# azuxmioy/Render-In-Between

Measured on AMD Instinct MI355X. Metric: rendered frames/sec at 512x512 (generator forward + blend, device-resident), higher is better.
Workload: dtype f32

## Files before the change

### render-in-between_amd/csrc/kernels.hip.h

```cpp
#pragma once
#include "igemm.hip.h"

namespace rib {

struct GemmDmaParams {
  const float* A; const float* B; float* C;
  int M, N, K, lda, ldc;
  size_t sA, sB, sC;
  int modB;
  int K2; unsigned long long kmask;
};

typedef uint32_t u32x4 __attribute__((ext_vector_type(4)));
__device__ __forceinline__ void split3_bf16(const float4 p, const float4 q, bf16x8& hi, bf16x8& mid, bf16x8& lo) {
  const float x[8] = {p.x, p.y, p.z, p.w, q.x, q.y, q.z, q.w};
  u32x4 h, m, l;
#pragma unroll
  for (int i = 0; i < 4; ++i) {
    const uint32_t u0 = __float_as_uint(x[2 * i]), u1 = __float_as_uint(x[2 * i + 1]);
    h[i] = __builtin_amdgcn_perm(u1, u0, 0x07060302u);
    const float r0 = x[2 * i] - __uint_as_float(u0 & 0xffff0000u), r1 = x[2 * i + 1] - __uint_as_float(u1 & 0xffff0000u);
    const uint32_t v0 = __float_as_uint(r0), v1 = __float_as_uint(r1);
    m[i] = __builtin_amdgcn_perm(v1, v0, 0x07060302u);
    const float s0 = r0 - __uint_as_float(v0 & 0xffff0000u), s1 = r1 - __uint_as_float(v1 & 0xffff0000u);
// ... 281 lines not shown
  const float* beta;
};

__device__ __forceinline__ void block_stats_64(const StatSrc& s, int n, int c0, int nch, double* red ,
                                               float* s_sc, float* s_sh) {
  const int j = threadIdx.x & 63, q = threadIdx.x >> 6;
  double a1 = 0.0, a2 = 0.0;
  if (j < nch) stats_from_partials(s.part + (size_t)n * s.tiles * 2 * s.Cs, s.tiles, s.Cs, c0 + j, q, 4, a1, a2);
  red[(q * 64 + j) * 2] = a1; red[(q * 64 + j) * 2 + 1] = a2;
  __syncthreads();
  if (q == 0 && j < nch) {
    double t1 = 0.0, t2 = 0.0;
#pragma unroll
    for (int k = 0; k < 4; ++k) { t1 += red[(k * 64 + j) * 2]; t2 += red[(k * 64 + j) * 2 + 1]; }
    float sc, sh;
    scale_shift_of(t1, t2, s.inv_count, s.gamma ? s.gamma[c0 + j] : 1.f, s.beta ? s.beta[c0 + j] : 0.f, sc, sh);
    s_sc[j] = sc; s_sh[j] = sh;
  }
  __syncthreads();
}

enum { WSRC_PLAIN = 0, WSRC_SPADE = 1, WSRC_JOIN = 2 };
struct WinoInParams {
  const float* x; int H, W, xC, Cin;
  const float* pro_scale; const float* pro_shift; int pro_ld, pro_lrelu;
  StatSrc st;
  float* v; int tilesY, tilesX;
  int nslices, ublocks;
  int x_ups; const float* slab; int slab_ld, col0; const float* sbias;
  const float* x2; const float* xres; float* o; const float* pro2_scale; const float* pro2_shift; StatSrc st2;
  int ldv;
  int nslices2, Cin2, xC2, x2_ups, lrelu2, pro2_ld;
  const float* slab2; int slab2_ld, col0_2; const float* sbias2;
};
__device__ __forceinline__ WinoInParams wino_second(const WinoInParams& p) {
  WinoInParams q = p;
  q.x = p.x2; q.xC = p.xC2; q.Cin = p.Cin2; q.x_ups = p.x2_ups; q.pro_lrelu = p.lrelu2;
  q.pro_scale = p.pro2_scale; q.pro_shift = p.pro2_shift; q.pro_ld = p.pro2_ld; q.st = p.st2;
  q.slab = p.slab2; q.slab_ld = p.slab2_ld; q.col0 = p.col0_2; q.sbias = p.sbias2;
  q.x2 = nullptr; q.v = p.v + p.Cin;
  return q;
}

__device__ __forceinline__ float spade_mod1(float x, float sc, float sh, float g, float bg, float b, float bb) {
  return fmaf(fmaf(x, sc, sh), 1.f + (g + bg), b + bb);
}

template <int MODE> struct WinoConsts { float4 sc, sh, bg, bb, sc2, sh2; bool aff; };
template <int MODE> struct WinoRaw { float4 a, b, c; };

template <int MODE>
__device__ __forceinline__ void wino_in_consts(const WinoInParams& p, int n, int slice, int c4, bool cok, double* red, float* s_sc,
                                               float* s_sh, WinoConsts<MODE>& k) {
  k.sc = make_float4(1.f, 1.f, 1.f, 1.f); k.sh = make_float4(0.f, 0.f, 0.f, 0.f);
  k.aff = false;
  const int l = (threadIdx.x & 15) * 4;
  if (p.st.part) {
    block_stats_64(p.st, n, slice * 64, min(64, p.Cin - slice * 64), red, s_sc, s_sh);
    k.sc = make_float4(s_sc[l], s_sc[l + 1], s_sc[l + 2], s_sc[l + 3]);
    k.sh = make_float4(s_sh[l], s_sh[l + 1], s_sh[l + 2], s_sh[l + 3]);
    k.aff = true;
  } else if (p.pro_scale && cok) {
    k.sc = *reinterpret_cast<const float4*>(p.pro_scale + (size_t)n * p.pro_ld + c4 * 4);
    k.sh = *reinterpret_cast<const float4*>(p.pro_shift + (size_t)n * p.pro_ld + c4 * 4);
    k.aff = true;
  }
// ... 128 lines not shown
  int nslices, ublocks;
};

__device__ __forceinline__ void wino_out_partials(double (*red)[256][4], const double s1[4], const double s2[4], double* stat_part,
                                                  int n, int ublocks, int ub, int slice, int CoutPad) {
#pragma unroll
  for (int e = 0; e < 4; ++e) { red[0][threadIdx.x][e] = s1[e]; red[1][threadIdx.x][e] = s2[e]; }
  __syncthreads();
  if (threadIdx.x < 64) {
    const int c = slice * 64 + threadIdx.x;
    if (c < CoutPad) {
      const int g = threadIdx.x >> 2, e = threadIdx.x & 3;
      double a1 = 0.0, a2 = 0.0;
#pragma unroll
      for (int s = 0; s < 16; ++s) { a1 += red[0][s * 16 + g][e]; a2 += red[1][s * 16 + g][e]; }
      double* dst = stat_part + (((size_t)n * ublocks + ub) * 2) * CoutPad;
      dst[c] = a1;
      dst[CoutPad + c] = a2;
    }
  }
}

__global__ __launch_bounds__(256) void k_wino_out(const WinoOutParams p) {
  __shared__ __attribute__((aligned(16))) double red[2][256][4];
  const int c4n = p.CoutPad / 4;
  const int slice = blockIdx.x % p.nslices, ub = blockIdx.x / p.nslices;
  const int c4 = slice * 16 + (threadIdx.x & 15);
  const int n = blockIdx.y;
  const int ntiles = p.tilesY * p.tilesX;
  double s1[4] = {0.0, 0.0, 0.0, 0.0}, s2[4] = {0.0, 0.0, 0.0, 0.0};
  if (c4 < c4n) {
    const float4 bv = *reinterpret_cast<const float4*>(p.bias + c4 * 4);
    const size_t plane = (size_t)ntiles * p.CoutPad;
    for (int u = ub * 16 + (threadIdx.x >> 4); u < ntiles * 2; u += p.ublocks * 16) {
      const int r = u & 1, tile = u >> 1;
      const float* mb = p.m + (size_t)n * 16 * plane + (size_t)tile * p.CoutPad + c4 * 4;
      float4 mm[3][4];
#pragma unroll
      for (int a = 0; a < 3; ++a)
#pragma unroll
        for (int q = 0; q < 4; ++q) mm[a][q] = *reinterpret_cast<const float4*>(mb + (size_t)((r + a) * 4 + q) * plane);
      const float sg = r ? -1.f : 1.f;
      float4 uu[4];
#pragma unroll
      for (int q = 0; q < 4; ++q)
        uu[q] = make_float4(mm[0][q].x + sg * (mm[1][q].x + mm[2][q].x), mm[0][q].y + sg * (mm[1][q].y + mm[2][q].y),
                            mm[0][q].z + sg * (mm[1][q].z + mm[2][q].z), mm[0][q].w + sg * (mm[1][q].w + mm[2][q].w));
      float4 yv[2];
      yv[0] = RIB_F4_ADD(RIB_F4_ADD(uu[0], uu[1]), uu[2]);
      yv[1] = RIB_F4_SUB(RIB_F4_SUB(uu[1], uu[2]), uu[3]);
      const int ty = tile / p.tilesX, tx = tile % p.tilesX;
      const int oy = 2 * ty + r;
      float rr[2][4];
#pragma unroll
      for (int q = 0; q < 2; ++q) {
        const int cy = min(oy, p.Hout - 1), cx = min(2 * tx + q, p.Wout - 1);
#pragma unroll
        for (int e = 0; e < 4; ++e)
          rr[q][e] = p.res ? p.res[(((size_t)n * p.Hout + cy) * p.Wout + cx) * p.resC + min(c4 * 4 + e, p.resC - 1)] : 0.f;
      }
#pragma unroll
      for (int q = 0; q < 2; ++q) {
        const int ox = 2 * tx + q;
        const bool inb = oy < p.Hout && ox < p.Wout;
        const float v4[4] = {yv[q].x + bv.x, yv[q].y + bv.y, yv[q].z + bv.z, yv[q].w + bv.w};
#pragma unroll
        for (int e = 0; e < 4; ++e) {
          float t = apply_act(v4[e] + rr[q][e], p.act);
          const bool ok = inb && c4 * 4 + e < p.Cout;
          if (ok) p.y[(((size_t)n * p.Hout + oy) * p.Wout + ox) * p.yC + p.yoff + c4 * 4 + e] = t;
          t = ok ? t : 0.f;
          s1[e] += (double)t; s2[e] += (double)t * (double)t;
        }
      }
    }
  }
  if (p.stat_part) wino_out_partials(red, s1, s2, p.stat_part, n, p.ublocks, ub, slice, p.CoutPad);
}

__device__ __constant__ float kWino4BT[6][6] = {
    {81.f / 64, 0.f, -45.f / 16, 0.f, 1.f, 0.f},        {0.f, -27.f / 16, -9.f / 4, 3.f / 4, 1.f, 0.f},
    {0.f, 27.f / 16, -9.f / 4, -3.f / 4, 1.f, 0.f},     {0.f, -27.f / 32, -9.f / 16, 3.f / 2, 1.f, 0.f},
    {0.f, 27.f / 32, -9.f / 16, -3.f / 2, 1.f, 0.f},    {0.f, 81.f / 64, 0.f, -45.f / 16, 0.f, 1.f}};
__device__ __constant__ float kWino4AT[4][6] = {
    {1.f, 1.f, 1.f, 1.f, 1.f, 0.f},                      {0.f, 3.f / 4, -3.f / 4, 3.f / 2, -3.f / 2, 0.f},
    {0.f, 9.f / 16, 9.f / 16, 9.f / 4, 9.f / 4, 0.f},    {0.f, 27.f / 64, -27.f / 64, 27.f / 8, -27.f / 8, 1.f}};

__device__ __forceinline__ float4 f4_fma(float a, float4 x, float4 acc) {
  return make_float4(fmaf(a, x.x, acc.x), fmaf(a, x.y, acc.y), fmaf(a, x.z, acc.z), fmaf(a, x.w, acc.w));
}
__device__ __forceinline__ float4 f4_scale(float a, float4 x) { return make_float4(a * x.x, a * x.y, a * x.z, a * x.w); }

// ... 58 lines not shown
          t[q] = f4_fma(coef, w, t[q]);
        }
      }
    }
    const size_t plane = (size_t)ntiles * p.ldv;
    float* vb = p.v + (size_t)n * 36 * plane + (size_t)tile * p.ldv + c4 * 4;
    const float4 ev1 = f4_fma(-9.f / 4, t[2], t[4]), od1 = f4_fma(-27.f / 16, t[1], f4_scale(3.f / 4, t[3]));
    const float4 ev2 = f4_fma(-9.f / 16, t[2], t[4]), od2 = f4_fma(-27.f / 32, t[1], f4_scale(3.f / 2, t[3]));
    if constexpr (!SC) {
      const float4 e24 = f4_fma(-45.f / 16, t[2], t[4]);
      const float4 o13 = f4_fma(-45.f / 16, t[3], t[5]);
      *reinterpret_cast<float4*>(vb + (size_t)(r * 6 + 0) * plane) = f4_fma(81.f / 64, t[0], e24);
      *reinterpret_cast<float4*>(vb + (size_t)(r * 6 + 5) * plane) = f4_fma(81.f / 64, t[1], o13);
    }
    *reinterpret_cast<float4*>(vb + (size_t)(r * 6 + 1) * plane) = RIB_F4_ADD(ev1, od1);
    *reinterpret_cast<float4*>(vb + (size_t)(r * 6 + 2) * plane) = RIB_F4_SUB(ev1, od1);
    *reinterpret_cast<float4*>(vb + (size_t)(r * 6 + 3) * plane) = RIB_F4_ADD(ev2, od2);
    *reinterpret_cast<float4*>(vb + (size_t)(r * 6 + 4) * plane) = RIB_F4_SUB(ev2, od2);
  }
}

template <int MODE, int MODE2 = -1>
__global__ __launch_bounds__(256) void k_wino4_in(const WinoInParams p) {
  __shared__ double red[4 * 64 * 2];
  __shared__ float s_sc[64], s_sh[64];
  const int slice = blockIdx.x % p.nslices, ub = blockIdx.x / p.nslices;
  if constexpr (MODE2 >= 0) {
    const int n1 = p.nslices - p.nslices2;
    if (slice >= n1) { wino4_in_slice<MODE2, true>(wino_second(p), slice - n1, ub, red, s_sc, s_sh); return; }
  }
  wino4_in_slice<MODE, false>(p, slice, ub, red, s_sc, s_sh);
}

__global__ __launch_bounds__(256) void k_wino4_out(const WinoOutParams p) {
  __shared__ __attribute__((aligned(16))) double red[2][256][4];
  const int c4n = p.CoutPad / 4;
  const int slice = blockIdx.x % p.nslices, ub = blockIdx.x / p.nslices;
  const int c4 = slice * 16 + (threadIdx.x & 15);
  const int n = blockIdx.y;
  const int ntiles = p.tilesY * p.tilesX;
  double s1[4] = {0.0, 0.0, 0.0, 0.0}, s2[4] = {0.0, 0.0, 0.0, 0.0};
  if (c4 < c4n) {
    const float4 bv = *reinterpret_cast<const float4*>(p.bias + c4 * 4);
    const size_t plane = (size_t)ntiles * p.CoutPad;
    for (int unit = ub * 16 + (threadIdx.x >> 4); unit < ntiles * 4; unit += p.ublocks * 16) {
      const int tile = unit >> 2, r = unit & 3;
      const float* mb = p.m + (size_t)n * 36 * plane + (size_t)tile * p.CoutPad + c4 * 4;
      float4 u[6];
#pragma unroll
      for (int q = 0; q < 6; ++q) u[q] = make_float4(0.f, 0.f, 0.f, 0.f);
      const int ax = r == 0 ? 0 : 5;
      const float cx_ = (r == 0 || r == 3) ? 1.f : 0.f;
      float4 mm[5][6];
#pragma unroll
      for (int k = 0; k < 5; ++k)
#pragma unroll
        for (int q = 0; q < 6; ++q) mm[k][q] = *reinterpret_cast<const float4*>(mb + (size_t)((k < 4 ? k + 1 : ax) * 6 + q) * plane);
#pragma unroll
      for (int k = 0; k < 5; ++k) {
        const float coef = k < 4 ? kWino4AT[r][k + 1] : cx_;
#pragma unroll
        for (int q = 0; q < 6; ++q) u[q] = f4_fma(coef, mm[k][q], u[q]);
      }
      const float4 s12 = RIB_F4_ADD(u[1], u[2]);
      const float4 d12 = RIB_F4_SUB(u[1], u[2]);
      const float4 s34 = RIB_F4_ADD(u[3], u[4]);
      const float4 d34 = RIB_F4_SUB(u[3], u[4]);
      float4 yv[4];
      yv[0] = make_float4(u[0].x + s12.x + s34.x, u[0].y + s12.y + s34.y, u[0].z + s12.z + s34.z, u[0].w + s12.w + s34.w);
      yv[1] = f4_fma(3.f / 4, d12, f4_scale(3.f / 2, d34));
      yv[2] = f4_fma(9.f / 16, s12, f4_scale(9.f / 4, s34));
      yv[3] = f4_fma(27.f / 64, d12, f4_fma(27.f / 8, d34, u[5]));
      const int ty = tile / p.tilesX, tx = tile % p.tilesX;
      const int oy = 4 * ty + r;
      float rr[4][4];
#pragma unroll
      for (int q = 0; q < 4; ++q) {
        const int cy = min(oy, p.Hout - 1), cx = min(4 * tx + q, p.Wout - 1);
#pragma unroll
        for (int e = 0; e < 4; ++e)
          rr[q][e] = p.res ? p.res[(((size_t)n * p.Hout + cy) * p.Wout + cx) * p.resC + min(c4 * 4 + e, p.resC - 1)] : 0.f;
      }
#pragma unroll
      for (int q = 0; q < 4; ++q) {
        const int ox = 4 * tx + q;
        const bool inb = oy < p.Hout && ox < p.Wout;
        const float v4[4] = {yv[q].x + bv.x, yv[q].y + bv.y, yv[q].z + bv.z, yv[q].w + bv.w};
#pragma unroll
        for (int e = 0; e < 4; ++e) {
          float t = apply_act(v4[e] + rr[q][e], p.act);
          const bool ok = inb && c4 * 4 + e < p.Cout;
          if (ok) p.y[(((size_t)n * p.Hout + oy) * p.Wout + ox) * p.yC + p.yoff + c4 * 4 + e] = t;
          t = ok ? t : 0.f;
          s1[e] += (double)t; s2[e] += (double)t * (double)t;
        }
      }
    }
  }
  if (p.stat_part) wino_out_partials(red, s1, s2, p.stat_part, n, p.ublocks, ub, slice, p.CoutPad);
}
#undef RIB_F4_SUB
#undef RIB_F4_ADD

struct ModulateParams {
  const float* slab; int ksplit, B, slab_ld, col0;
  const float* bias;
  const float* xm; int xmC, xm_ups;
  const float* m_scale; const float* m_shift; int m_ld;
  StatSrc st;
  int C, nsets;
  float* ys0; float* ys1; int act0, act1;
  int Hout, Wout;
  int nslices, pblocks;
};
// ... 611 lines not shown
```

### render-in-between_amd/csrc/rib.hip

```cpp
#include "kernels.hip.h"
#include "rib_host.h"
#include <hip/hip_ext.h>

#include <algorithm>
#include <array>
#include <climits>
#include <cmath>
#include <cstdio>
#include <cstdlib>
#include <cstring>
#include <map>
#include <memory>
#include <string>
#include <variant>
#include <vector>


#include "variants.hip.h"
#define RIB_V(sec, ...) RIB_I_V(RIB_F_EXTERN, __VA_ARGS__)
#define RIB_VK(sec, ...) RIB_I_VK(RIB_F_EXTERN, __VA_ARGS__)
#define RIB_VT(sec, ...) RIB_I_VT(RIB_F_EXTERN, __VA_ARGS__)
#define RIB_VTK(sec, ...) RIB_I_VTK(RIB_F_EXTERN, __VA_ARGS__)
#define RIB_V9(sec, ...) RIB_I_V9(RIB_F_EXTERN, __VA_ARGS__)
#define RIB_VU4(sec, ...) RIB_I_VU4(RIB_F_EXTERN, __VA_ARGS__)
// ... 365 lines not shown
  }
  return best;
}

enum OpKind { OP_PACK, OP_IGEMM, OP_FINALIZE, OP_POOL, OP_INADD, OP_SPLITEPI, OP_MODULATE, OP_WINO_IN, OP_WINO_OUT, OP_LOWC, OP_GEMM };

enum PtrSpace { PS_NULL = 0, PS_WS, PS_WEIGHT, PS_USER, PS_WINO };
enum UserSlot { U_LABEL = 0, U_FAKE, U_PREV, U_IMG, U_MASK, U_FUSE, U_COUNT };
struct PRef {
  PtrSpace sp = PS_NULL;
  size_t off = 0;
};


using OpParams = std::variant<PackParams, IgemmParams, FinalizeParams, PoolParams, InAddParams, SplitEpiParams, ModulateParams,
                              WinoInParams, WinoOutParams, LowcParams, GemmDmaParams>;
static_assert(std::is_same<std::variant_alternative_t<OP_IGEMM, OpParams>, IgemmParams>::value &&
              std::is_same<std::variant_alternative_t<OP_GEMM, OpParams>, GemmDmaParams>::value, "OpParams follows OpKind");
struct Op {
  int kclass = 0;
  std::string name;
  std::string for_op;
  bool label_only = false;
  dim3 grid;
  double flops = 0;
  const Variant* var = nullptr;
  int small_co = 0;
  bool head = false;
  bool fuse_blend = false;
  bool wino = false;
  int wino_m = 0;
  int wi_mode = 0;
  int wi_mode2 = -1;
  int lowc_ce = 0, lowc_ncol = 0, lowc_tw = 32;
  OpParams params;
  struct Binding { PRef ref; unsigned field = 0; };
  static constexpr int kMaxBindings = 24;
  Binding binds[kMaxBindings];
  int nbinds = 0;

  OpKind kind() const { return (OpKind)params.index(); }
  template <class P> const P& as() const { return std::get<P>(params); }
  template <class P, class T> unsigned field_of(T* P::*f) const {
    return (unsigned)(reinterpret_cast<const char*>(&(as<P>().*f)) - reinterpret_cast<const char*>(&params));
  }
  template <class P, class T> unsigned field_of(StatSrc P::*s, T* StatSrc::*f) const {
    return (unsigned)(reinterpret_cast<const char*>(&((as<P>().*s).*f)) - reinterpret_cast<const char*>(&params));
  }
  PRef ref_at(unsigned field) const {
    for (int i = 0; i < nbinds; ++i) if (binds[i].field == field) return binds[i].ref;
    return PRef();
  }
  void bind_at(unsigned field, PRef r) {
    int i = 0;
    while (i < nbinds && binds[i].field != field) ++i;
    if (r.sp == PS_NULL) { if (i < nbinds) binds[i] = binds[--nbinds]; return; }
    if (i == kMaxBindings) abort();
    binds[i] = Binding{r, field};
    if (i == nbinds) ++nbinds;
  }
  template <class P, class T> bool bound(T* P::*f) const { return ref_at(field_of(f)).sp != PS_NULL; }
};
template <class P> struct OpOf : Op {
  OpOf(int kclass_, const std::string& name_) { kclass = kclass_; name = name_; memset(&params.emplace<P>(), 0, sizeof(P)); }
  P& p() { return std::get<P>(params); }
  template <class T> void bind(T* P::*f, PRef r) { bind_at(field_of(f), r); }
// ... 337 lines not shown
    } else {
      add(p + ".weight", {c.cout, c.cin, c.ks, c.ks}, c.used);
      add(p + ".bias", {c.cout}, c.used);
    }
    if (c.in_affine) {
      add(c.name + ".layers.norm.weight", {c.cout}, c.used);
      add(c.name + ".layers.norm.bias", {c.cout}, c.used);
    }
  }
}

const std::vector<float>* tensor_data(rib_handle* h, const std::string& name) {
  auto it = h->tensor_index.find(name);
  if (it == h->tensor_index.end()) return nullptr;
  TensorDef& t = h->tensors[it->second];
  return t.set ? &t.data : nullptr;
}

struct FusionPolicy {
  bool consumer_stats = !getenv("RIB_NO_CONSUMER_STATS");
  bool head_conv = !getenv("RIB_NO_HEADCONV");
  bool small_conv = !getenv("RIB_NO_SMALLCONV");
  long wino_max_px = getenv("RIB_WINO_MAX_PX") ? atol(getenv("RIB_WINO_MAX_PX")) : 16384;
  int wino_force = getenv("RIB_WINO_M") ? atoi(getenv("RIB_WINO_M")) : 0;
  bool split_k = !getenv("RIB_NO_SPLITK");
  bool n16 = !getenv("RIB_NO_N16");
  int lowc_tw = getenv("RIB_LOWC_TW") ? (atoi(getenv("RIB_LOWC_TW")) == 16 ? 16 : 32) : 0;
  long cond_gemm_max_px = getenv("RIB_COND_GEMM_MAX_PX") ? atol(getenv("RIB_COND_GEMM_MAX_PX")) : 4096;
  bool unfused_spade = !getenv("RIB_NO_UNFUSED_SPADE");
  bool lazy_sources = !getenv("RIB_NO_LAZY");
  bool fuse_shortcut = !getenv("RIB_NO_FUSE_SHORTCUT");
  bool wino_shortcut = !getenv("RIB_NO_WINO_SHORTCUT");
  int wino_shortcut_m = getenv("RIB_WINO_SHORTCUT_M") ? atoi(getenv("RIB_WINO_SHORTCUT_M")) : 0;
  bool ws_reuse = !getenv("RIB_NO_WS_REUSE");
  static bool pair_mask_encoders() { return !getenv("RIB_NO_PAIR"); }
};

struct Builder {
  rib_handle* h;
  Plan* P;
  int B;
  const FusionPolicy pol;
  size_t ws = 0;
  std::string error;
  bool mark_label = false;
  bool pair_mask = false;
  bool defer_stats = true;
  void materialize(const Norm& n, const std::string& consumer = std::string()) {
    if (n.pend && !n.pend->pushed) { n.pend->pushed = true; n.pend->fin.for_op = consumer; push(n.pend->fin); }
  }
  static bool has_partials(const Norm& n) { return n.pend && !n.pend->pushed; }
  void finalize_or_defer(Op& f, Norm* out, bool now, size_t part_off, int tiles, int Cs, float inv_count, bool affine, size_t g_off, size_t be_off) {
    if (now || !pol.consumer_stats || !defer_stats || mark_label || tiles > STATS_MAX_PARTIALS) { push(f); return; }
    auto ps = std::make_shared<PendingStats>();
    ps->fin = f; ps->part_off = part_off; ps->tiles = tiles; ps->Cs = Cs; ps->inv_count = inv_count;
    ps->affine = affine; ps->g_off = g_off; ps->be_off = be_off;
    out->pend = ps;
  }
  template <class P> bool take_partials(const Norm& n, OpOf<P>& op, StatSrc P::*src) {
    if (!has_partials(n) || n.pend->tiles > STATS_MAX_PARTIALS) return false;
    const PendingStats& ps = *n.pend;
    StatSrc& st = op.p().*src;
    st.tiles = ps.tiles; st.Cs = ps.Cs; st.inv_count = ps.inv_count;
    op.bind(src, &StatSrc::part, WS(ps.part_off));
    if (ps.affine) { op.bind(src, &StatSrc::gamma, WT(ps.g_off)); op.bind(src, &StatSrc::beta, WT(ps.be_off)); }
    return true;
// ... 243 lines not shown
    }
    return true;
  }

  bool conv_lowc(const ConvArgs& a, const std::string& opname) {
    const ConvDef& c = *a.cd;
    const int H = a.in.H, W = a.in.W;
    if (!c.wl_off || c.ks != 3 || c.stride != 1 || a.ups || a.pro || a.res || a.aux || a.y_nchw.sp != PS_NULL || a.y_user.sp != PS_NULL ||
        a.in.uc[0] + a.in.uc[1] + a.in.uc[2] != c.cin) { error = opname + ": not a layer k_conv_lowc can run"; return false; }
    if (a.out.H != H || a.out.W != W) { error = fmt("%s: output size mismatch", opname.c_str()); return false; }
    OpOf<LowcParams> op(RIB_KC_IGEMM, opname); op.lowc_ce = c.lowc_ce; op.lowc_ncol = c.lowc_ncol;
    LowcParams& p = op.p();
    p.c0 = a.in.uc[0]; p.c1 = a.in.uc[1]; p.c2 = a.in.uc[2];
    p.H = H; p.W = W; p.yC = a.out.Cp; p.yoff = a.yoff; p.Cout = a.cout_store >= 0 ? a.cout_store : h->padc(c.cout);
    p.act = a.act; p.CoutPad = c.coutp;
    const int tw = pol.lowc_tw ? pol.lowc_tw : ((c.lowc_ncol == 64 && !a.want_stats) ? 16 : 32);
    op.lowc_tw = tw;
    p.tilesX = (W + tw - 1) / tw; p.tilesY = (H + 7) / 8;
    if (p.Cout > c.lowc_ncol || c.cout > c.lowc_ncol) { error = opname + ": more output columns than the k_conv_lowc instantiation has"; return false; }
    op.bind(&LowcParams::s0, US(a.in.usrc[0])); if (p.c1) op.bind(&LowcParams::s1, US(a.in.usrc[1])); if (p.c2) op.bind(&LowcParams::s2, US(a.in.usrc[2]));
    op.bind(&LowcParams::w, WT(c.wl_off)); op.bind(&LowcParams::bias, WT(c.b_off)); op.bind(&LowcParams::y, WS(a.out.off));
    const int tiles = p.tilesX * p.tilesY;
    size_t part_off = 0;
    if (a.want_stats) { part_off = alloc((size_t)B * tiles * 2 * c.coutp * sizeof(double)); op.bind(&LowcParams::stat_part, WS(part_off)); }
    op.grid = dim3(tiles, B, 1);
    op.flops = 2.0 * c.cin * 9.0 * c.cout * (double)H * W * B;
    P->flops[RIB_KC_IGEMM] += op.flops;
    push(op);
    if (a.want_stats) {
      OpOf<FinalizeParams> f = finalize_op(opname, part_off, tiles, c.coutp, h->padc(c.cout), *a.stats_out, a.stats_choff, H, W, a.affine ? &c : nullptr, B);
      finalize_or_defer(f, a.stats_out, a.stats_choff != 0 || a.stats_now, part_off, tiles, c.coutp, f.p().inv_count, a.affine, c.g_off, c.be_off);
    }
    return true;
  }

  bool conv_wino(const ConvArgs& a, const std::string& opname, int Hout, int Wout) {
    const ConvDef& c = *a.cd;
    const int wino_force = pol.wino_force;
    const int wm = a.aux ? shortcut_wino_m(c, *a.aux, opname, Hout, Wout) : (wino_force == 2 || wino_force == 4 ? wino_force : default_wino_m(Hout, Wout));
    const int NP = (wm + 2) * (wm + 2);
    const int tilesY = (Hout + wm - 1) / wm, tilesX = (Wout + wm - 1) / wm, ntiles = tilesY * tilesX;
    const std::string gname = opname + (wm == 2 ? ".wino" : ".wino4");
    const int K2 = a.aux ? a.aux->cinp : 0, ldv = c.cinp + K2;
    unsigned long long kmask = 0;
    if (a.aux) {
      if (a.aux_in.Cp != K2 || a.aux_in.H != Hout || a.aux_in.W != Wout || a.in.H != Hout || a.in.W != Wout) { error = opname + ": fused shortcut operand does not fit"; return false; }
      for (int r = 1; r <= wm; ++r) for (int q = 1; q <= wm; ++q) kmask |= 1ull << (r * (wm + 2) + q);
    }
    const size_t v_off = alloc((size_t)B * NP * ntiles * ldv * sizeof(float));
    const size_t m_off = alloc((size_t)B * NP * ntiles * c.coutp * sizeof(float));
    {
      OpOf<WinoInParams> op(RIB_KC_CONVAUX, opname + ".wino_in"); op.for_op = gname; op.wino_m = wm;
      WinoInParams& wi = op.p();
      wi.H = a.in.H; wi.W = a.in.W; wi.xC = a.in.Cp; wi.Cin = c.cinp; wi.tilesY = tilesY; wi.tilesX = tilesX;
      wi.pro_lrelu = a.pro_lrelu ? 1 : 0; wi.ldv = ldv;
      op.bind(&WinoInParams::x, WS(a.in.off)); op.bind(&WinoInParams::v, WS(v_off));
      if (a.in.lazy) {
        const LazySrc& L = *a.in.lazy;
        if (a.pro || a.pro_lrelu) { error = gname + ": a lazy input carries its own prologue"; return false; }
        op.wi_mode = L.mode;
        op.bind(&WinoInParams::x, WS(L.x.off)); wi.xC = L.x.Cp;
        wi.pro_ld = L.nx.ld;
        if (!take_partials(L.nx, op, &WinoInParams::st)) { materialize(L.nx, gname); op.bind(&WinoInParams::pro_scale, WS(L.nx.sc)); op.bind(&WinoInParams::pro_shift, WS(L.nx.sh)); }
        if (L.mode == WSRC_SPADE) {
          wi.x_ups = L.x_ups ? 1 : 0; wi.pro_lrelu = L.lrelu ? 1 : 0;
          op.bind(&WinoInParams::slab, WS(L.slab_off)); wi.slab_ld = L.slab_ld; wi.col0 = L.col0; op.bind(&WinoInParams::sbias, WT(L.sbias_off));
        } else {
          if (L.has2) {
            op.bind(&WinoInParams::x2, WS(L.x2.off));
            if (L.n2.ld != L.nx.ld) { error = gname + ": join operands with different statistics rows"; return false; }
            if (!take_partials(L.n2, op, &WinoInParams::st2)) { materialize(L.n2, gname); op.bind(&WinoInParams::pro2_scale, WS(L.n2.sc)); op.bind(&WinoInParams::pro2_shift, WS(L.n2.sh)); }
          } else op.bind(&WinoInParams::xres, WS(L.xres.off));
          op.bind(&WinoInParams::o, WS(L.o.off));
        }
      } else if (a.pro && !(a.pro_choff == 0 && take_partials(*a.pro, op, &WinoInParams::st))) {
        materialize(*a.pro, gname);
        wi.pro_ld = a.pro->ld;
        op.bind(&WinoInParams::pro_scale, WS(a.pro->sc + a.pro_choff * sizeof(float))); op.bind(&WinoInParams::pro_shift, WS(a.pro->sh + a.pro_choff * sizeof(float)));
      }
      if (a.aux) {
        if (op.wi_mode == WSRC_JOIN) { error = gname + ": a join cannot carry a second source"; return false; }
        wi.nslices2 = (K2 + 63) / 64; wi.Cin2 = K2; wi.xC2 = a.aux_in.Cp;
        op.wi_mode2 = WSRC_PLAIN;
        if (a.aux_in.lazy) {
          const LazySrc& L = *a.aux_in.lazy;
          if (L.mode != WSRC_SPADE) { error = gname + ": lazy shortcut input of an unknown kind"; return false; }
          op.wi_mode2 = WSRC_SPADE;
          op.bind(&WinoInParams::x2, WS(L.x.off)); wi.xC2 = L.x.Cp; wi.pro2_ld = L.nx.ld; wi.x2_ups = L.x_ups ? 1 : 0; wi.lrelu2 = L.lrelu ? 1 : 0;
          if (!take_partials(L.nx, op, &WinoInParams::st2)) { materialize(L.nx, gname); op.bind(&WinoInParams::pro2_scale, WS(L.nx.sc)); op.bind(&WinoInParams::pro2_shift, WS(L.nx.sh)); }
          op.bind(&WinoInParams::slab2, WS(L.slab_off)); wi.slab2_ld = L.slab_ld; wi.col0_2 = L.col0; op.bind(&WinoInParams::sbias2, WT(L.sbias_off));
        } else op.bind(&WinoInParams::x2, WS(a.aux_in.off));
      }
      const int nsl = (c.cinp + 63) / 64 + wi.nslices2, units = ntiles * (wm + 2);
      wi.nslices = nsl; wi.ublocks = std::max(1, std::min((units + 15) / 16, (wi.st.tiles > 0 ? 512 : 4096) / nsl));
      op.grid = dim3(wi.ublocks * nsl, B, 1);
      push(op);
    }
    {
      Choice ch;
      ch.v = pick_gemm_dma(h->prec(), (long)TB_() * NP, ntiles, c.coutp, c.cinp);
      if (!ch.v) ch = choose_variant(h->prec(), 1, 1, false, false, c.coutp, TB_() * NP, tilesY, tilesX, c.cinp, false, 0, false);
      auto it = h->choices.find(fmt("%d,%d,%d|%s", TB_(), P->H, P->W, gname.c_str()));
      if (it != h->choices.end()) {
        const Variant& tv = kVariants[it->second.first];
        if (tv.BF16 != h->prec() || tv.KS != 1 || tv.STRIDE != 1 || tv.UPS || tv.SPADE || tv.NF == 0 || c.cinp % tv.BK != 0 || it->second.second != 1 || (a.aux && !tv.dma())) {
          error = fmt("%s: tuned choice (variant %d, ksplit %d) does not fit this layer", gname.c_str(), it->second.first, it->second.second); return false;
        }
        ch.v = &tv; ch.ksplit = 1;
      }
      const Variant* v = ch.v;
      if (!v) { error = gname + ": no 1x1 kernel variant"; return false; }
      if (a.aux && !v->dma()) { error = gname + ": the fused shortcut needs a k_gemm_dma tile"; return false; }
      const int set = ensure_wino_set(h, (int)(&c - h->convs.data()), wm, a.aux ? (int)(a.aux - h->convs.data()) : -1);
      if (set < 0) { error = gname + ": " + h->err; return false; }
      const double fl = 2.0 * c.cin * 9.0 * c.cout * (double)Hout * Wout * B + (a.aux ? 2.0 * a.aux->cin * a.aux->cout * (double)Hout * Wout * B : 0.0);
      P->flops[RIB_KC_IGEMM] += fl;
      if (v->dma()) {
        OpOf<GemmDmaParams> op(RIB_KC_IGEMM, gname); op.var = v; op.wino = true; op.wino_m = wm; op.flops = fl;
        GemmDmaParams& g = op.p();
        g.M = ntiles; g.N = c.coutp; g.K = c.cinp; g.lda = ldv; g.ldc = c.coutp;
        g.sA = (size_t)ntiles * ldv; g.sB = (size_t)c.coutp * ldv; g.sC = (size_t)ntiles * c.coutp; g.modB = NP;
        g.K2 = K2; g.kmask = kmask;
        op.bind(&GemmDmaParams::A, WS(v_off)); op.bind(&GemmDmaParams::B, WINO(set)); op.bind(&GemmDmaParams::C, WS(m_off));
        op.grid = dim3((ntiles + v->BM() - 1) / v->BM(), (c.coutp + v->BN() - 1) / v->BN(), B * NP);
        push(op);
      } else {
      OpOf<IgemmParams> op(RIB_KC_IGEMM, gname); op.var = v; op.wino = true; op.wino_m = wm; op.flops = fl;
// ... 731 lines not shown
        IgemmParams& p = std::get<IgemmParams>(params);
        p.zeros = R.blob + h->zero_off;
        if (op.small_co > 0 && op.head) {
          if (op.fuse_blend && R.user[U_FUSE]) {
            p.bl_img = reinterpret_cast<const float*>(R.user[U_IMG]); p.bl_dain = reinterpret_cast<const float*>(R.user[U_FAKE]);
            p.bl_fuse = reinterpret_cast<float*>(const_cast<void*>(R.user[U_FUSE]));
          }
          launch_head(op.small_co, p.Cin, bf16, op.grid, st, p);
        } else if (op.small_co > 0) {
          const size_t lds = ((size_t)18 * 18 * (p.Cin + 4) + (size_t)op.small_co * 9 * p.Cin) * sizeof(float);
          switch (op.small_co) {
            case 1: launch_small_t<1>(bf16, op.grid, lds, st, p); break;
            case 2: launch_small_t<2>(bf16, op.grid, lds, st, p); break;
            case 3: launch_small_t<3>(bf16, op.grid, lds, st, p); break;
            default: launch_small_t<4>(bf16, op.grid, lds, st, p); break;
          }
        } else
        RIB_KLAUNCH(pick_igemm_fn(op.var, p), op.grid, dim3(256 * op.var->KW), 0, st, p);
      } break;
      case OP_GEMM:
        RIB_KLAUNCH(h->products == RIB_PRODUCTS_BF16X3 && op.var->gfn_x3 ? op.var->gfn_x3 : op.var->gfn, op.grid, dim3(256), 0, st, std::get<GemmDmaParams>(params));
        break;
      case OP_FINALIZE: {
        const FinalizeParams& p = std::get<FinalizeParams>(params);
        if (p.tiles > 512) RIB_KLAUNCH(k_stats_finalize<4>, dim3((p.Cs + 3) / 4, op.grid.y, op.grid.z), dim3(1024), 0, st, p);
        else RIB_KLAUNCH(k_stats_finalize<16>, op.grid, dim3(1024), 0, st, p);
      } break;
      case OP_MODULATE: RIB_LAUNCH_ST(bf16, k_spade_modulate, op.grid, dim3(256), 0, st, std::get<ModulateParams>(params)); break;
      case OP_SPLITEPI: RIB_LAUNCH_ST(bf16, k_splitk_epilogue, op.grid, dim3(256), 0, st, std::get<SplitEpiParams>(params)); break;
      case OP_POOL: RIB_LAUNCH_ST(bf16, k_avgpool, op.grid, dim3(256), 0, st, std::get<PoolParams>(params)); break;
      case OP_INADD: RIB_LAUNCH_ST(bf16, k_in_add, op.grid, dim3(256), 0, st, std::get<InAddParams>(params)); break;
      case OP_WINO_IN: {
        const WinoInParams& p = std::get<WinoInParams>(params);
        if (op.wi_mode2 >= 0) {
          const bool s1 = op.wi_mode == WSRC_SPADE, s2 = op.wi_mode2 == WSRC_SPADE;
#define RIB_WINO_IN2(K)                                                                                     \
          if (s1 && s2) RIB_KLAUNCH((K<WSRC_SPADE, WSRC_SPADE>), op.grid, dim3(256), 0, st, p);             \
          else if (s1) RIB_KLAUNCH((K<WSRC_SPADE, WSRC_PLAIN>), op.grid, dim3(256), 0, st, p);              \
          else if (s2) RIB_KLAUNCH((K<WSRC_PLAIN, WSRC_SPADE>), op.grid, dim3(256), 0, st, p);              \
          else RIB_KLAUNCH((K<WSRC_PLAIN, WSRC_PLAIN>), op.grid, dim3(256), 0, st, p)
          if (op.wino_m == 4) { RIB_WINO_IN2(k_wino4_in); } else { RIB_WINO_IN2(k_wino_in); }
#undef RIB_WINO_IN2
        } else if (op.wino_m == 4) {
          if (op.wi_mode == WSRC_SPADE) RIB_KLAUNCH(k_wino4_in<WSRC_SPADE>, op.grid, dim3(256), 0, st, p);
          else if (op.wi_mode == WSRC_JOIN) RIB_KLAUNCH(k_wino4_in<WSRC_JOIN>, op.grid, dim3(256), 0, st, p);
          else RIB_KLAUNCH(k_wino4_in<WSRC_PLAIN>, op.grid, dim3(256), 0, st, p);
        } else {
          if (op.wi_mode == WSRC_SPADE) RIB_KLAUNCH(k_wino_in<WSRC_SPADE>, op.grid, dim3(256), 0, st, p);
          else if (op.wi_mode == WSRC_JOIN) RIB_KLAUNCH(k_wino_in<WSRC_JOIN>, op.grid, dim3(256), 0, st, p);
          else RIB_KLAUNCH(k_wino_in<WSRC_PLAIN>, op.grid, dim3(256), 0, st, p);
        }
      } break;
      case OP_WINO_OUT:
        if (op.wino_m == 4) RIB_KLAUNCH(k_wino4_out, op.grid, dim3(256), 0, st, std::get<WinoOutParams>(params));
        else RIB_KLAUNCH(k_wino_out, op.grid, dim3(256), 0, st, std::get<WinoOutParams>(params));
        break;
      case OP_LOWC: launch_lowc(op.lowc_ce, op.lowc_ncol, op.lowc_tw, op.grid, st, std::get<LowcParams>(params)); break;
      case OP_PACK: RIB_LAUNCH_ST(bf16, k_pack, op.grid, dim3(256), 0, st, std::get<PackParams>(params)); break;
    }
  }
  g_prof_pair = ProfPair();
  if (h->profiling && !h->prof_kernels) {
    hipEvent_t e1 = nullptr;
    HIP_TRY(h, hipEventCreate(&e1));
    HIP_TRY(h, hipEventRecord(e1, st));
    h->prof_events.push_back({-1, e1});
  }
  HIP_TRY(h, hipGetLastError());
  return RIB_OK;
}

int check_ready(rib_handle* h) {
  if (!h) return RIB_ERR_INVALID;
  if (!h->weights_ready) return fail(h, RIB_ERR_STATE, "weights not loaded: call rib_finalize_weights() or rib_import_weights() first");
// ... 549 lines not shown
  const std::string key = blk + "." + (which == "s" ? std::string("0") : which);
  auto it = h->spade_index.find(key);
  if (it == h->spade_index.end()) return fail(h, RIB_ERR_INVALID, fmt("no SPADE group '%s'", key.c_str()));
  const SpadeGroup& sg = h->spades[it->second];
  const int set = which == "s" ? 1 : 0;
  const int condp = h->padc(sg.cond);
  for (int ch = 0; ch < sg.C; ++ch) {
    const int v = set * sg.Cp + ch;
    const int colg = (v / 32) * 64 + (v % 32), colb = colg + 32;
    for (int k = 0; k < sg.cond; ++k) {
      w_2c_by_cond[(size_t)ch * sg.cond + k] = h->host_blob[sg.w_off + (size_t)colg * condp + k];
      w_2c_by_cond[(size_t)(sg.C + ch) * sg.cond + k] = h->host_blob[sg.w_off + (size_t)colb * condp + k];
    }
    bias_2c[ch] = h->host_blob[sg.b_off + colg];
    bias_2c[sg.C + ch] = h->host_blob[sg.b_off + colb];
  }
  return RIB_OK;
}

static int launch_info_head(const Op& op, char* buf, size_t buflen) {
  if (op.kind() == OP_IGEMM && op.small_co > 0)
    snprintf(buf, buflen, "%s|%d|%u,%u,%u|%s 16x16 tile, %d output channels%s|%.0f", op.name.c_str(), op.kclass, op.grid.x, op.grid.y, op.grid.z,
             op.head ? "head (taps as MFMA columns)" : "direct (vector ALUs)", op.small_co, op.fuse_blend ? " + fused blend" : "", op.flops);
  else if (op.kind() == OP_IGEMM)
    snprintf(buf, buflen, "%s|%d|%u,%u,%u|tile %dx%d BN %d BK %d s%d k%d ups%d ksplit%d kw%d tb%d%s v%d|%.0f", op.name.c_str(), op.kclass, op.grid.x, op.grid.y, op.grid.z,
             op.var->TH(), op.var->TW(), op.var->BN(), op.var->BK, op.var->STRIDE, op.var->KS, (int)op.var->UPS, op.as<IgemmParams>().ksplit, op.var->KW, op.var->DMAK ? 100 + (op.var->TB == 9 ? 9 : 0) : op.var->TB,
             op.wino ? (op.wino_m == 4 ? " wino4" : " wino") : "", (int)(op.var - kVariants), op.flops);
  else if (op.kind() == OP_GEMM)
    snprintf(buf, buflen, "%s|%d|%u,%u,%u|gemm (LDS-DMA staged operands) tile %dx%d BK 32, %d x [%d x %d x %d]%s|%.0f", op.name.c_str(), op.kclass, op.grid.x, op.grid.y, op.grid.z,
             op.var->BM(), op.var->BN(), (int)op.grid.z, op.as<GemmDmaParams>().M, op.as<GemmDmaParams>().N, op.as<GemmDmaParams>().K, (std::string(op.wino ? (op.wino_m == 4 ? " wino4" : " wino") : "") + (op.as<GemmDmaParams>().K2 ? fmt(" + K %d of the 1x1 shortcut at %d positions", op.as<GemmDmaParams>().K2, __builtin_popcountll(op.as<GemmDmaParams>().kmask)) : std::string())).c_str(), op.flops);
  else if (op.kind() == OP_LOWC)
    snprintf(buf, buflen, "%s|%d|%u,%u,%u|lowc (caller's NCHW tensors, K = 9 x %d real channels) 8x%d tile, %d columns|%.0f", op.name.c_str(), op.kclass,
             op.grid.x, op.grid.y, op.grid.z, op.lowc_ce, op.lowc_tw, op.lowc_ncol, op.flops);
  else
    snprintf(buf, buflen, "%s|%d|%u,%u,%u||0", op.name.c_str(), op.kclass, op.grid.x, op.grid.y, op.grid.z);
  return RIB_OK;
}

static double op_algorithmic_bytes(const rib_handle* h, const Plan* P, const Op& op) {
  const double e = h->esz(), Bn = P->B;
  switch (op.kind()) {
    case OP_IGEMM: {
      const IgemmParams& p = op.as<IgemmParams>();
      const double samples = p.pair ? 2.0 * Bn : Bn;
      const int taps = op.var ? op.var->KS * op.var->KS : 9;
      double b = samples * p.Hin * p.Win * (double)p.Cin * e
                 + (double)p.CoutPad * taps * p.Cin * e * (p.pair ? 2.0 : 1.0)
                 + p.CoutPad * 4.0;
      if (op.var && op.var->SPADE) {
        b += Bn * p.Hout * p.Wout * (double)p.C * e / (p.xm_ups ? 4.0 : 1.0);
        b += Bn * p.Hout * p.Wout * (double)p.C * e * p.nsets;
      } else if (op.bound(&IgemmParams::slab)) {
        b += (double)p.ksplit * samples * p.Hout * p.Wout * p.CoutPad * 4.0;
      } else {
        b += samples * p.Hout * p.Wout * (double)p.Cout * (op.small_co > 0 || p.y_f32 ? 4.0 : e);
        if (op.bound(&IgemmParams::res)) b += samples * p.Hout * p.Wout * (double)p.Cout * e / (p.res_ups ? 4.0 : 1.0);
        if (op.bound(&IgemmParams::x2)) b += samples * p.Hout * p.Wout * (double)p.Cin2 * e + (double)p.CoutPad * p.Cin2 * e;
        if (op.fuse_blend) b += Bn * p.Hout * p.Wout * 3.0 * 4.0 * 3.0;
      }
      return b;
    }
    case OP_GEMM: {
      const GemmDmaParams& g = op.as<GemmDmaParams>();
      const double Z = op.grid.z;
      const double z2 = g.K2 ? Bn * __builtin_popcountll(g.kmask) : 0.0, nb2 = g.K2 ? (double)__builtin_popcountll(g.kmask) : 0.0;
      return Z * g.M * (double)g.K * e + (g.modB ? (double)g.modB : 1.0) * g.N * (double)g.K * e + Z * g.M * (double)g.N * 4.0 +
             z2 * g.M * (double)g.K2 * e + nb2 * g.N * (double)g.K2 * e;
// ... 195 lines not shown
```

Measured before the change: 398.7.

## Stage Winograd input patches in LDS and vectorize residual loads

Adds LDS-staged Winograd input-transform kernels, on by default. Each workgroup fetches and normalises a block of overlapping tile pixels once into shared memory, then computes the B^T d B transforms from LDS. Before, every tile row re-fetched and re-normalised its overlapping neighbours from global memory. A host heuristic picks the block shape to balance workgroup count against halo overhead. The output-transform kernels also load the residual as one float4 when alignment allows, instead of four scalar loads. The trade-off is extra LDS use and a barrier per block, which may lower occupancy.

```diff
diff --git a/render-in-between_amd/csrc/kernels.hip.h b/render-in-between_amd/csrc/kernels.hip.h
--- a/render-in-between_amd/csrc/kernels.hip.h
+++ b/render-in-between_amd/csrc/kernels.hip.h
@@ -337,6 +337,7 @@
   int ldv;
   int nslices2, Cin2, xC2, x2_ups, lrelu2, pro2_ld;
   const float* slab2; int slab2_ld, col0_2; const float* sbias2;
+  int bty, btx, nbx;
 };
 __device__ __forceinline__ WinoInParams wino_second(const WinoInParams& p) {
   WinoInParams q = p;
@@ -531,6 +532,7 @@
   if (c4 < c4n) {
     const float4 bv = *reinterpret_cast<const float4*>(p.bias + c4 * 4);
     const size_t plane = (size_t)ntiles * p.CoutPad;
+    const bool res4 = p.res && p.resC % 4 == 0 && c4 * 4 + 3 < p.resC;
     for (int u = ub * 16 + (threadIdx.x >> 4); u < ntiles * 2; u += p.ublocks * 16) {
       const int r = u & 1, tile = u >> 1;
       const float* mb = p.m + (size_t)n * 16 * plane + (size_t)tile * p.CoutPad + c4 * 4;
@@ -554,9 +556,14 @@
 #pragma unroll
       for (int q = 0; q < 2; ++q) {
         const int cy = min(oy, p.Hout - 1), cx = min(2 * tx + q, p.Wout - 1);
-#pragma unroll
-        for (int e = 0; e < 4; ++e)
-          rr[q][e] = p.res ? p.res[(((size_t)n * p.Hout + cy) * p.Wout + cx) * p.resC + min(c4 * 4 + e, p.resC - 1)] : 0.f;
+        const float* rp = p.res + (((size_t)n * p.Hout + cy) * p.Wout + cx) * p.resC;
+        if (res4) {
+          const float4 r4 = *reinterpret_cast<const float4*>(rp + c4 * 4);
+          rr[q][0] = r4.x; rr[q][1] = r4.y; rr[q][2] = r4.z; rr[q][3] = r4.w;
+        } else {
+#pragma unroll
+          for (int e = 0; e < 4; ++e) rr[q][e] = p.res ? rp[min(c4 * 4 + e, p.resC - 1)] : 0.f;
+        }
       }
 #pragma unroll
       for (int q = 0; q < 2; ++q) {
@@ -681,6 +688,124 @@
   wino4_in_slice<MODE, false>(p, slice, ub, red, s_sc, s_sh);
 }
 
+#ifndef RIB_WINO_LDS_EARLY
+#define RIB_WINO_LDS_EARLY 1
+#endif
+constexpr int WINO_LDS_MAXPX = 128;
+
+template <int MODE, bool SC, int M>
+__device__ __forceinline__ void wino_in_slice_lds(const WinoInParams& p, int slice, int blk, double* red, float* s_sc, float* s_sh, float4* patch) {
+  constexpr int HALO = SC ? 0 : 1, T = M + 2, NR = SC ? M : T, Q0 = SC ? 1 : 0, Q1 = SC ? T - 1 : T;
+  constexpr int NPASS = WINO_LDS_MAXPX / 16;
+  const int c4n = p.Cin / 4;
+  const int n = blockIdx.y;
+  const int lane = threadIdx.x & 15, slot = threadIdx.x >> 4;
+  const int c4 = slice * 16 + lane;
+  const bool cok = c4 < c4n;
+  const int ty0 = (blk / p.nbx) * p.bty, tx0 = (blk % p.nbx) * p.btx;
+  const int PW = M * p.btx + 2 * HALO, npix = (M * p.bty + 2 * HALO) * PW;
+  const int y0 = M * ty0 - HALO, x0 = M * tx0 - HALO;
+  WinoConsts<MODE> kc;
+  if (!RIB_WINO_LDS_EARLY) wino_in_consts<MODE>(p, n, slice, c4, cok, red, s_sc, s_sh, kc);
+  WinoRaw<MODE> raw[NPASS];
+#pragma unroll
+  for (int i = 0; i < NPASS; ++i) {
+    const int pp = slot + 16 * i;
+    if (cok && pp < npix) {
+      const int ly = pp / PW, lx = pp - ly * PW;
+      wino_fetch<MODE>(p, n, min(max(y0 + ly, 0), p.H - 1), min(max(x0 + lx, 0), p.W - 1), c4, raw[i]);
+    }
+  }
+  if (RIB_WINO_LDS_EARLY) wino_in_consts<MODE>(p, n, slice, c4, cok, red, s_sc, s_sh, kc);
+#pragma unroll
+  for (int i = 0; i < NPASS; ++i) {
+    const int pp = slot + 16 * i;
+    if (cok && pp < npix) {
+      const int ly = pp / PW, lx = pp - ly * PW;
+      const int iy = y0 + ly, ix = x0 + lx;
+      const bool inb = iy >= 0 && iy < p.H && ix >= 0 && ix < p.W;
+      float4 w = wino_value<MODE>(p, kc, raw[i]);
+      if constexpr (MODE == WSRC_JOIN) {
+        if (inb && ly >= HALO && ly < M * p.bty + HALO && lx >= HALO && lx < M * p.btx + HALO)
+          *reinterpret_cast<float4*>(p.o + (((size_t)n * p.H + iy) * p.W + ix) * p.xC + c4 * 4) = w;
+      }
+      if (!inb) w = make_float4(0.f, 0.f, 0.f, 0.f);
+      patch[pp * 16 + lane] = w;
+    }
+  }
+  __syncthreads();
+  if (!cok) return;
+  const int ntiles = p.tilesY * p.tilesX;
+  const int nunits = p.bty * p.btx * NR;
+  const size_t plane = (size_t)ntiles * p.ldv;
+  for (int u = slot; u < nunits; u += 16) {
+    const int r = (SC ? 1 : 0) + u % NR, lt = u / NR;
+    const int lty = lt / p.btx, ltx = lt - lty * p.btx;
+    const int ty = ty0 + lty, tx = tx0 + ltx;
+    if (ty >= p.tilesY || tx >= p.tilesX) continue;
+    const int tile = ty * p.tilesX + tx;
+    const int d0 = ((M * lty - (1 - HALO)) * PW + M * ltx - (1 - HALO)) * 16 + lane;
+    float* vb = p.v + (size_t)n * (T * T) * plane + (size_t)tile * p.ldv + c4 * 4;
+    if constexpr (M == 2) {
+      const int ia = r == 0 ? 0 : (r == 2 ? 2 : 1), ib = r == 0 ? 2 : (r == 1 ? 2 : (r == 2 ? 1 : 3));
+      const float sg = r == 1 ? 1.f : -1.f;
+      float4 t[4];
+#pragma unroll
+      for (int q = Q0; q < Q1; ++q) {
+        const float4 v0 = patch[d0 + (ia * PW + q) * 16], v1 = patch[d0 + (ib * PW + q) * 16];
+        t[q] = make_float4(v0.x + sg * v1.x, v0.y + sg * v1.y, v0.z + sg * v1.z, v0.w + sg * v1.w);
+      }
+      if constexpr (!SC) *reinterpret_cast<float4*>(vb + (size_t)(r * 4 + 0) * plane) = RIB_F4_SUB(t[0], t[2]);
+      *reinterpret_cast<float4*>(vb + (size_t)(r * 4 + 1) * plane) = RIB_F4_ADD(t[1], t[2]);
+      *reinterpret_cast<float4*>(vb + (size_t)(r * 4 + 2) * plane) = RIB_F4_SUB(t[2], t[1]);
+      if constexpr (!SC) *reinterpret_cast<float4*>(vb + (size_t)(r * 4 + 3) * plane) = RIB_F4_SUB(t[1], t[3]);
+    } else {
+      const int a0 = r == 0 ? 0 : 1, da = (r == 0 || r == 5) ? 2 : 1, na = (r == 0 || r == 5) ? 3 : 4;
+      float4 t[6];
+#pragma unroll
+      for (int q = 0; q < 6; ++q) t[q] = make_float4(0.f, 0.f, 0.f, 0.f);
+#pragma unroll
+      for (int k = 0; k < 4; ++k) {
+        if (k < na) {
+          const int a = a0 + k * da;
+          const float coef = kWino4BT[r][a];
+#pragma unroll
+          for (int q = Q0; q < Q1; ++q) t[q] = f4_fma(coef, patch[d0 + (a * PW + q) * 16], t[q]);
+        }
+      }
+      const float4 ev1 = f4_fma(-9.f / 4, t[2], t[4]), od1 = f4_fma(-27.f / 16, t[1], f4_scale(3.f / 4, t[3]));
+      const float4 ev2 = f4_fma(-9.f / 16, t[2], t[4]), od2 = f4_fma(-27.f / 32, t[1], f4_scale(3.f / 2, t[3]));
+      if constexpr (!SC) {
+        const float4 e24 = f4_fma(-45.f / 16, t[2], t[4]);
+        const float4 o13 = f4_fma(-45.f / 16, t[3], t[5]);
+        *reinterpret_cast<float4*>(vb + (size_t)(r * 6 + 0) * plane) = f4_fma(81.f / 64, t[0], e24);
+        *reinterpret_cast<float4*>(vb + (size_t)(r * 6 + 5) * plane) = f4_fma(81.f / 64, t[1], o13);
+      }
+      *reinterpret_cast<float4*>(vb + (size_t)(r * 6 + 1) * plane) = RIB_F4_ADD(ev1, od1);
+      *reinterpret_cast<float4*>(vb + (size_t)(r * 6 + 2) * plane) = RIB_F4_SUB(ev1, od1);
+      *reinterpret_cast<float4*>(vb + (size_t)(r * 6 + 3) * plane) = RIB_F4_ADD(ev2, od2);
+      *reinterpret_cast<float4*>(vb + (size_t)(r * 6 + 4) * plane) = RIB_F4_SUB(ev2, od2);
+    }
+  }
+}
+
+template <int M, int MODE, int MODE2>
+__device__ __forceinline__ void wino_in_lds_body(const WinoInParams& p) {
+  __shared__ double red[4 * 64 * 2];
+  __shared__ float s_sc[64], s_sh[64];
+  __shared__ float4 patch[WINO_LDS_MAXPX * 16];
+  const int slice = blockIdx.x % p.nslices, blk = blockIdx.x / p.nslices;
+  if constexpr (MODE2 >= 0) {
+    const int n1 = p.nslices - p.nslices2;
+    if (slice >= n1) { wino_in_slice_lds<MODE2, true, M>(wino_second(p), slice - n1, blk, red, s_sc, s_sh, patch); return; }
+  }
+  wino_in_slice_lds<MODE, false, M>(p, slice, blk, red, s_sc, s_sh, patch);
+}
+template <int MODE, int MODE2 = -1>
+__global__ __launch_bounds__(256) void k_wino_in_lds(const WinoInParams p) { wino_in_lds_body<2, MODE, MODE2>(p); }
+template <int MODE, int MODE2 = -1>
+__global__ __launch_bounds__(256) void k_wino4_in_lds(const WinoInParams p) { wino_in_lds_body<4, MODE, MODE2>(p); }
+
 __global__ __launch_bounds__(256) void k_wino4_out(const WinoOutParams p) {
   __shared__ __attribute__((aligned(16))) double red[2][256][4];
   const int c4n = p.CoutPad / 4;
@@ -692,6 +817,7 @@
   if (c4 < c4n) {
     const float4 bv = *reinterpret_cast<const float4*>(p.bias + c4 * 4);
     const size_t plane = (size_t)ntiles * p.CoutPad;
+    const bool res4 = p.res && p.resC % 4 == 0 && c4 * 4 + 3 < p.resC;
     for (int unit = ub * 16 + (threadIdx.x >> 4); unit < ntiles * 4; unit += p.ublocks * 16) {
       const int tile = unit >> 2, r = unit & 3;
       const float* mb = p.m + (size_t)n * 36 * plane + (size_t)tile * p.CoutPad + c4 * 4;
@@ -726,9 +852,14 @@
 #pragma unroll
       for (int q = 0; q < 4; ++q) {
         const int cy = min(oy, p.Hout - 1), cx = min(4 * tx + q, p.Wout - 1);
-#pragma unroll
-        for (int e = 0; e < 4; ++e)
-          rr[q][e] = p.res ? p.res[(((size_t)n * p.Hout + cy) * p.Wout + cx) * p.resC + min(c4 * 4 + e, p.resC - 1)] : 0.f;
+        const float* rp = p.res + (((size_t)n * p.Hout + cy) * p.Wout + cx) * p.resC;
+        if (res4) {
+          const float4 r4 = *reinterpret_cast<const float4*>(rp + c4 * 4);
+          rr[q][0] = r4.x; rr[q][1] = r4.y; rr[q][2] = r4.z; rr[q][3] = r4.w;
+        } else {
+#pragma unroll
+          for (int e = 0; e < 4; ++e) rr[q][e] = p.res ? rp[min(c4 * 4 + e, p.resC - 1)] : 0.f;
+        }
       }
 #pragma unroll
       for (int q = 0; q < 4; ++q) {
diff --git a/render-in-between_amd/csrc/rib.hip b/render-in-between_amd/csrc/rib.hip
--- a/render-in-between_amd/csrc/rib.hip
+++ b/render-in-between_amd/csrc/rib.hip
@@ -421,6 +421,7 @@
   int wino_m = 0;
   int wi_mode = 0;
   int wi_mode2 = -1;
+  bool wi_lds = false;
   int lowc_ce = 0, lowc_ncol = 0, lowc_tw = 32;
   OpParams params;
   struct Binding { PRef ref; unsigned field = 0; };
@@ -824,6 +825,7 @@
   bool fuse_shortcut = !getenv("RIB_NO_FUSE_SHORTCUT");
   bool wino_shortcut = !getenv("RIB_NO_WINO_SHORTCUT");
   int wino_shortcut_m = getenv("RIB_WINO_SHORTCUT_M") ? atoi(getenv("RIB_WINO_SHORTCUT_M")) : 0;
+  bool wino_in_lds = !getenv("RIB_NO_WINO_IN_LDS");
   bool ws_reuse = !getenv("RIB_NO_WS_REUSE");
   static bool pair_mask_encoders() { return !getenv("RIB_NO_PAIR"); }
 };
@@ -1133,6 +1135,24 @@
       finalize_or_defer(f, a.stats_out, a.stats_choff != 0 || a.stats_now, part_off, tiles, c.coutp, f.p().inv_count, a.affine, c.g_off, c.be_off);
     }
     return true;
+  }
+
+  void wino_in_block(int wm, int tilesY, int tilesX, int nsl, int& bty, int& btx) const {
+    long best_wg = -1, best_px = 0;
+    bty = btx = 1;
+    for (int y = 1; y <= std::min(tilesY, 8); ++y)
+      for (int x = 1; x <= std::min(tilesX, 16); ++x) {
+        if ((wm * y + 2) * (wm * x + 2) > WINO_LDS_MAXPX) continue;
+        const long nb = (long)((tilesY + y - 1) / y) * ((tilesX + x - 1) / x);
+        const long wg = nb * nsl * B, px = nb * (wm * y + 2) * (wm * x + 2);
+        const bool full = wg >= 256, best_full = best_wg >= 256;
+        bool better;
+        if (best_wg < 0) better = true;
+        else if (full != best_full) better = full;
+        else if (full) better = px < best_px;
+        else better = wg > best_wg || (wg == best_wg && px < best_px);
+        if (better) { best_wg = wg; best_px = px; bty = y; btx = x; }
+      }
   }
 
   bool conv_wino(const ConvArgs& a, const std::string& opname, int Hout, int Wout) {
@@ -1194,6 +1214,11 @@
       }
       const int nsl = (c.cinp + 63) / 64 + wi.nslices2, units = ntiles * (wm + 2);
       wi.nslices = nsl; wi.ublocks = std::max(1, std::min((units + 15) / 16, (wi.st.tiles > 0 ? 512 : 4096) / nsl));
+      if (pol.wino_in_lds) {
+        wino_in_block(wm, tilesY, tilesX, nsl, wi.bty, wi.btx);
+        wi.nbx = (tilesX + wi.btx - 1) / wi.btx; wi.ublocks = ((tilesY + wi.bty - 1) / wi.bty) * wi.nbx;
+        op.wi_lds = true;
+      }
       op.grid = dim3(wi.ublocks * nsl, B, 1);
       push(op);
     }
@@ -1991,6 +2016,17 @@
       case OP_INADD: RIB_LAUNCH_ST(bf16, k_in_add, op.grid, dim3(256), 0, st, std::get<InAddParams>(params)); break;
       case OP_WINO_IN: {
         const WinoInParams& p = std::get<WinoInParams>(params);
+        if (op.wi_lds && op.wi_mode2 < 0) {
+          if (op.wino_m == 4) {
+            if (op.wi_mode == WSRC_SPADE) RIB_KLAUNCH(k_wino4_in_lds<WSRC_SPADE>, op.grid, dim3(256), 0, st, p);
+            else if (op.wi_mode == WSRC_JOIN) RIB_KLAUNCH(k_wino4_in_lds<WSRC_JOIN>, op.grid, dim3(256), 0, st, p);
+            else RIB_KLAUNCH(k_wino4_in_lds<WSRC_PLAIN>, op.grid, dim3(256), 0, st, p);
+          } else {
+            if (op.wi_mode == WSRC_SPADE) RIB_KLAUNCH(k_wino_in_lds<WSRC_SPADE>, op.grid, dim3(256), 0, st, p);
+            else if (op.wi_mode == WSRC_JOIN) RIB_KLAUNCH(k_wino_in_lds<WSRC_JOIN>, op.grid, dim3(256), 0, st, p);
+            else RIB_KLAUNCH(k_wino_in_lds<WSRC_PLAIN>, op.grid, dim3(256), 0, st, p);
+          }
+        } else
         if (op.wi_mode2 >= 0) {
           const bool s1 = op.wi_mode == WSRC_SPADE, s2 = op.wi_mode2 == WSRC_SPADE;
 #define RIB_WINO_IN2(K)                                                                                     \
@@ -1998,7 +2034,8 @@
           else if (s1) RIB_KLAUNCH((K<WSRC_SPADE, WSRC_PLAIN>), op.grid, dim3(256), 0, st, p);              \
           else if (s2) RIB_KLAUNCH((K<WSRC_PLAIN, WSRC_SPADE>), op.grid, dim3(256), 0, st, p);              \
           else RIB_KLAUNCH((K<WSRC_PLAIN, WSRC_PLAIN>), op.grid, dim3(256), 0, st, p)
-          if (op.wino_m == 4) { RIB_WINO_IN2(k_wino4_in); } else { RIB_WINO_IN2(k_wino_in); }
+          if (op.wi_lds) { if (op.wino_m == 4) { RIB_WINO_IN2(k_wino4_in_lds); } else { RIB_WINO_IN2(k_wino_in_lds); } }
+          else if (op.wino_m == 4) { RIB_WINO_IN2(k_wino4_in); } else { RIB_WINO_IN2(k_wino_in); }
 #undef RIB_WINO_IN2
         } else if (op.wino_m == 4) {
           if (op.wi_mode == WSRC_SPADE) RIB_KLAUNCH(k_wino4_in<WSRC_SPADE>, op.grid, dim3(256), 0, st, p);
@@ -2614,7 +2651,20 @@
   else if (op.kind() == OP_LOWC)
     snprintf(buf, buflen, "%s|%d|%u,%u,%u|lowc (caller's NCHW tensors, K = 9 x %d real channels) 8x%d tile, %d columns|%.0f", op.name.c_str(), op.kclass,
              op.grid.x, op.grid.y, op.grid.z, op.lowc_ce, op.lowc_tw, op.lowc_ncol, op.flops);
-  else
+  else if (op.kind() == OP_WINO_IN && op.wi_lds) {
+    const WinoInParams& w = op.as<WinoInParams>();
+    auto src = [](int mode, bool stats, bool ups, bool lrelu) {
+      std::string s = mode == WSRC_SPADE ? "spade" : (mode == WSRC_JOIN ? "join" : "plain"), f;
+      if (mode == WSRC_PLAIN && stats) f = "statistics";
+      if (mode == WSRC_SPADE && ups) f = "2x upsampled";
+      if (mode != WSRC_JOIN && lrelu) f += std::string(f.empty() ? "" : " and ") + "LeakyReLU";
+      return f.empty() ? s : s + " (" + f + ")";
+    };
+    std::string d = src(op.wi_mode, op.bound(&WinoInParams::pro_scale) || op.ref_at(op.field_of(&WinoInParams::st, &StatSrc::part)).sp != PS_NULL, w.x_ups != 0, w.pro_lrelu != 0);
+    if (op.wi_mode2 >= 0) d += " + second " + src(op.wi_mode2, false, w.x2_ups != 0, w.lrelu2 != 0);
+    snprintf(buf, buflen, "%s|%d|%u,%u,%u|staged in LDS: blocks of %dx%d F(%dx%d) tiles, %dx%d px patch, %s|0", op.name.c_str(), op.kclass, op.grid.x, op.grid.y, op.grid.z,
+             w.bty, w.btx, op.wino_m, op.wino_m, op.wino_m * w.bty + 2, op.wino_m * w.btx + 2, d.c_str());
+  } else
     snprintf(buf, buflen, "%s|%d|%u,%u,%u||0", op.name.c_str(), op.kclass, op.grid.x, op.grid.y, op.grid.z);
   return RIB_OK;
 }
```

Measured after the change: 402.6 (median of 6 runs). No clear change (+1.0%).
